# HansBambel/SmaAt-UNet

Hardware: NVIDIA H100
Metric: SmaAt-UNet fwd frames/sec @ B=32 12×288×288; depthwise % HBM roofline (higher is better)
Workload: dtype f32

## Files before the change

### smaat_unet_b200/csrc/dsconv_fused.cu

```cuda
#include <stdlib.h>

#include <type_traits>

#include "tc_common.cuh"

namespace smaat {

struct DsParams {
  const float* dw_w;
  const float* dw_b;
  const float* scale;
  const float* shift;
  float* y;
  int64_t y_bstride;
  double* stats;
  const float* oc_w;
  const float* oc_b;
  float* oc_y;
  const float* gate_sc;
  float* pool_sum;
  float* pool_max;
  float* pooled;
  int pooled_bf16;
  int npart;
// ... 301 lines not shown
        static_assert(GPC % 2 == 0, "fragment sets alternate within a chunk");
        const unsigned char* ast = nullptr;
        uint64_t bd = 0, bl = 0;
        AFrags<PREC, KS> fa, fb;
        auto step = [&](int i, int hf, int part, AFrags<PREC, KS>& cur, AFrags<PREC, KS>& prev) {
          if (part == 0) {
            if (hf == 0) {
              const int sa = gc % AS;
              mbar_wait(&a_full[sa], (gc / AS) & 1u);
              ast = a_base + sa * L::AST_BYTES;
            }
            wait_b(NW * gc + hf, bd, bl);
          }
          load_a_frags<PREC, KS>(ast, part * KS, t, m0, m1, cur);
          if (hf == 0) mma_a_frags<N_TILE, PREC, KS>(acc[0], cur, bd, bl, part * KS);
          else mma_a_frags<N_TILE, PREC, KS>(acc[NA - 1], cur, bd, bl, part * KS);
          wgmma_wait<1>();
          wgmma_keep(prev);
          if (part == 0) {
            if (hf == 1) release_b(NW * gc);
            else if (i > 0) release(gc - 1);
          }
        };
        for (int i = 0; i < nch; ++i, ++gc) {
#pragma unroll
          for (int hf = 0; hf < NW; ++hf) {
#pragma unroll
            for (int part = 0; part < GPC; part += 2) {
              step(i, hf, part, fa, fb);
              step(i, hf, part + 1, fb, fa);
            }
          }
        }
        wgmma_wait0();
        wgmma_keep(fa);
        wgmma_keep(fb);
      } else {
        constexpr int KS = L::KS, GPC = (TC_BK / 8) / KS;
        const unsigned char* ast = nullptr;
        uint64_t bd0 = 0, bl0 = 0;
        auto group = [&](AFrags<PREC, KS>(&cur)[NH], AFrags<PREC, KS>(&prev)[NH], int q) {
          const int part = q % GPC;
          if (part == 0) wait_stages(ast, bd0, bl0);
#pragma unroll
          for (int h = 0; h < NH; ++h) load_a_frags<PREC, KS>(ast + h * L::A_BYTES, part * KS, t, m0, m1, cur[h]);
          mma_a_frags<N_TILE, PREC, KS, NH>(acc, cur, bd0, bl0, part * KS);
          wgmma_wait<1>();
#pragma unroll
          for (int h = 0; h < NH; ++h) wgmma_keep(prev[h]);
          if (part == 0 && q > 0) release(gc - 1);
          if (part == GPC - 1) ++gc;
        };
        AFrags<PREC, KS> fa[NH], fb[NH];
        const int ngrp = nch * GPC;
        int q = 0;
        for (; q + 1 < ngrp; q += 2) {
          group(fa, fb, q);
          group(fb, fa, q + 1);
        }
        if (q < ngrp) group(fa, fb, q);
        wgmma_wait0();
#pragma unroll
        for (int h = 0; h < NH; ++h) {
          wgmma_keep(fa[h]);
          wgmma_keep(fb[h]);
        }
      }
#pragma unroll
      for (int h = 0; h < NA; ++h) wgmma_keep(acc[h]);
      release(gc - 1);

#pragma unroll
      for (int h = 0; h < NA; ++h) {
        float (&ac)[N_TILE / 2] = acc[h];
        const int hp = WIDE ? 0 : h;
        const int n0 = (np * NW + (WIDE ? h : 0)) * N_TILE;
        const int y_org = ty * TH + hp * PH;
        const int gy0 = y_org + m0 / PW, gx0 = tx * PW + m0 % PW;
        const int gy1 = y_org + m1 / PW, gx1 = tx * PW + m1 % PW;
        const bool v0 = gy0 < p.H && gx0 < p.W, v1 = gy1 < p.H && gx1 < p.W;
        const int64_t o0 = (int64_t)gy0 * p.W + gx0, o1 = (int64_t)gy1 * p.W + gx1;
        if (!WIDE && p.stats) {
          const double npix = (double)((__popc(__ballot_sync(0xffffffffu, v0)) + __popc(__ballot_sync(0xffffffffu, v1))) / 4);
#pragma unroll
          for (int j = 0; j < N_TILE / 8; ++j) {
#pragma unroll
            for (int e = 0; e < 2; ++e) {
              const float a = v0 ? ac[4 * j + e] : 0.f, bb = v1 ? ac[4 * j + 2 + e] : 0.f;
              const float s1 = frag_colsum(a + bb), s2 = frag_colsum(fmaf(a, a, bb * bb));
              const int c = 8 * j + 2 * t + e;
              if (lane < 4 && c < p.Cout) {
                const double sc = (double)aff[c], sh = (double)aff[L::AFF_N + c];
                atomicAdd(p.stats + c, sc * (double)s1 + npix * sh);
                atomicAdd(p.stats + p.Cout + c, sc * sc * (double)s2 + 2.0 * sc * sh * (double)s1 + npix * sh * sh);
              }
            }
          }
        }
        if (!WIDE && p.ncls) {
#pragma unroll
          for (int j = 0; j < N_TILE / 8; ++j) {
#pragma unroll
            for (int e = 0; e < 2; ++e) {
              const int c = 8 * j + 2 * t + e;
              const float sc = aff[c], sh = aff[L::AFF_N + c];
              ac[4 * j + e] = fmaxf(fmaf(ac[4 * j + e], sc, sh), act_lo);
              ac[4 * j + 2 + e] = fmaxf(fmaf(ac[4 * j + 2 + e], sc, sh), act_lo);
            }
          }
          float best0 = -INFINITY, best1 = -INFINITY;
          int arg0 = 0, arg1 = 0;
#pragma unroll 1
          for (int cl = 0; cl < p.ncls; ++cl) {
            const float* wr = cls_w + cl * N_TILE + 2 * t;
            float d0 = 0.f, d1 = 0.f;
#pragma unroll
            for (int j = 0; j < N_TILE / 8; ++j) {
              const float2 w = *reinterpret_cast<const float2*>(wr + 8 * j);
              d0 = fmaf(ac[4 * j], w.x, d0);
              d1 = fmaf(ac[4 * j + 2], w.x, d1);
              d0 = fmaf(ac[4 * j + 1], w.y, d0);
              d1 = fmaf(ac[4 * j + 3], w.y, d1);
            }
            d0 += __shfl_xor_sync(0xffffffffu, d0, 1);
            d0 += __shfl_xor_sync(0xffffffffu, d0, 2);
            d1 += __shfl_xor_sync(0xffffffffu, d1, 1);
            d1 += __shfl_xor_sync(0xffffffffu, d1, 2);
            const float ob = cls_b[cl];
            const float l0 = d0 + ob, l1 = d1 + ob;
            if (best0 == best0 && (l0 > best0 || l0 != l0)) { best0 = l0; arg0 = cl; }
            if (best1 == best1 && (l1 > best1 || l1 != l1)) { best1 = l1; arg1 = cl; }
            if (p.oc_y && t == (cl & 3)) {
              TA* yk = reinterpret_cast<TA*>(p.oc_y) + ((int64_t)b * p.ncls + cl) * P;
              if (v0) st_act(yk + o0, l0);
              if (v1) st_act(yk + o1, l1);
            }
          }
          if (p.cls) {
            if (v0 && t == 0) p.cls[(int64_t)b * P + o0] = arg0;
            if (v1 && t == 1) p.cls[(int64_t)b * P + o1] = arg1;
          }
        } else if (!WIDE && p.oc_y) {
          float d0 = 0.f, d1 = 0.f;
#pragma unroll
          for (int j = 0; j < N_TILE / 8; ++j) {
#pragma unroll
            for (int e = 0; e < 2; ++e) {
              const int c = 8 * j + 2 * t + e;
              const float sc = aff[c], sh = aff[L::AFF_N + c], w = aff[2 * L::AFF_N + c];
              d0 = fmaf(fmaxf(fmaf(ac[4 * j + e], sc, sh), act_lo), w, d0);
              d1 = fmaf(fmaxf(fmaf(ac[4 * j + 2 + e], sc, sh), act_lo), w, d1);
            }
          }
          d0 += __shfl_xor_sync(0xffffffffu, d0, 1);
          d0 += __shfl_xor_sync(0xffffffffu, d0, 2);
          d1 += __shfl_xor_sync(0xffffffffu, d1, 1);
          d1 += __shfl_xor_sync(0xffffffffu, d1, 2);
          const float ob = p.oc_b ? __ldg(p.oc_b) : 0.f;
          if (t == 0) {
            TA* oy = reinterpret_cast<TA*>(p.oc_y) + (int64_t)b * P;
            if (v0) st_act(oy + o0, d0 + ob);
            if (v1) st_act(oy + o1, d1 + ob);
          }
        } else if (L::ST_BUFS) {
          const int y_half = y_org + wg * (PH / 2);
#pragma unroll
          for (int s = 0; s < N_TILE / 32; ++s) {
            if (n0 + 32 * s >= p.Cout) break;
            const uint32_t buf = st_base + (st_n % L::ST_BUFS) * L::ST_BOX;
            if (st_leader) bulk_wait_read<L::ST_BUFS - 1>();
            wg_sync(2 + wg);
#pragma unroll
            for (int jj = 0; jj < 4; ++jj) {
              const int j = 4 * s + jj;
              float v[4];
#pragma unroll
              for (int q = 0; q < 4; ++q) v[q] = (t & 2) ? ac[4 * j + (q ^ 2)] : ac[4 * j + q];
              quad_transpose(v, quad);
              const int c = n0 + 8 * j + st_ch;
              const float sc = aff[c], sh = aff[L::AFF_N + c];
              const float4 o = make_float4(fmaxf(fmaf(v[0], sc, sh), act_lo), fmaxf(fmaf(v[1], sc, sh), act_lo),
                                           fmaxf(fmaf(v[2], sc, sh), act_lo), fmaxf(fmaf(v[3], sc, sh), act_lo));
              if constexpr (BA) {
                asm volatile("st.shared.v2.b32 [%0], {%1, %2};" ::"r"(buf + st_off + 1024u * jj), "r"(f32x2_bf16x2(o.x, o.y)),
                             "r"(f32x2_bf16x2(o.z, o.w))
                             : "memory");
              } else {
                asm volatile("st.shared.v4.f32 [%0], {%1, %2, %3, %4};" ::"r"(buf + st_off + 2048u * jj), "f"(o.x), "f"(o.y),
                             "f"(o.z), "f"(o.w)
                             : "memory");
              }
            }
            fence_proxy_async_smem();
            wg_sync(2 + wg);
            if (st_leader) {
              tma_store_4d(&map_y, buf, tx * PW, y_half, n0 + 32 * s, b);
              bulk_commit();
            }
            if (p.pooled) {
              const bool parts = !BA && p.pool_sum;
              const int pt = threadIdx.x & 127, pch = pt >> 2, pq = pt & 3;
              const int c = n0 + 32 * s + pch;
              float psum = 0.f, pmax = -INFINITY;
#pragma unroll
              for (int it = 0; it < 2; ++it) {
                constexpr int NQ = PW / 4;
                const int item = pq + 4 * it, rp = item / NQ, qd = item % NQ;
                const int px = 2 * rp * PW + 4 * qd;
                float4 u, v;
                if constexpr (BA) {
                  const uint32_t a0 = (uint32_t)(pch * 128 + px * 2), a1 = a0 + (uint32_t)(PW * 2);
                  uint2 hu, hv;
                  asm volatile("ld.shared.v2.b32 {%0, %1}, [%2];" : "=r"(hu.x), "=r"(hu.y) : "r"(buf + a0));
                  asm volatile("ld.shared.v2.b32 {%0, %1}, [%2];" : "=r"(hv.x), "=r"(hv.y) : "r"(buf + a1));
                  u = bf16x4_f32(hu);
                  v = bf16x4_f32(hv);
                } else {
                  const uint32_t a0 = (uint32_t)(pch * 256 + px * 4), a1 = a0 + (uint32_t)(PW * 4);
                  asm volatile("ld.shared.v4.f32 {%0, %1, %2, %3}, [%4];" : "=f"(u.x), "=f"(u.y), "=f"(u.z), "=f"(u.w)
                               : "r"(buf + (a0 ^ (((a0 >> 7) & SW_MASK) << 4))));
                  asm volatile("ld.shared.v4.f32 {%0, %1, %2, %3}, [%4];" : "=f"(v.x), "=f"(v.y), "=f"(v.z), "=f"(v.w)
                               : "r"(buf + (a1 ^ (((a1 >> 7) & SW_MASK) << 4))));
                }
                const int gy = y_half + 2 * rp, gx = tx * PW + 4 * qd;
                const bool in0 = gx < p.W && gy < p.H, in1 = gx < p.W && gy + 1 < p.H;
                if (parts && in0) {
                  psum += (u.x + u.y) + (u.z + u.w);
                  pmax = fmaxf(pmax, fmaxf(fmaxf(u.x, u.y), fmaxf(u.z, u.w)));
                }
                if (in1) {
                  if (parts) {
                    psum += (v.x + v.y) + (v.z + v.w);
                    pmax = fmaxf(pmax, fmaxf(fmaxf(v.x, v.y), fmaxf(v.z, v.w)));
                  }
                  if (c < p.Cout) {
                    const int hw = p.W >> 1;
                    const int64_t o = ((int64_t)b * p.Cout + c) * (int64_t)(p.H >> 1) * hw + (int64_t)(gy >> 1) * hw + (gx >> 1);
                    const float2 m2 = make_float2(fmaxf(fmaxf(u.x, u.y), fmaxf(v.x, v.y)), fmaxf(fmaxf(u.z, u.w), fmaxf(v.z, v.w)));
                    if (BA && p.pooled_bf16)
                      *reinterpret_cast<uint32_t*>(reinterpret_cast<uint16_t*>(p.pooled) + o) = f32x2_bf16x2(m2.x, m2.y);
                    else
                      *reinterpret_cast<float2*>(p.pooled + o) = m2;
                  }
                }
              }
              if (parts) {
                psum += __shfl_xor_sync(0xffffffffu, psum, 1);
                psum += __shfl_xor_sync(0xffffffffu, psum, 2);
                pmax = fmaxf(pmax, __shfl_xor_sync(0xffffffffu, pmax, 1));
                pmax = fmaxf(pmax, __shfl_xor_sync(0xffffffffu, pmax, 2));
                if (pq == 0 && c < p.Cout) {
                  const int64_t o = ((int64_t)b * p.npart + 2 * ((ty * NH + hp) * p.tiles_x + tx) + wg) * p.Cout + c;
                  p.pool_sum[o] = psum;
                  p.pool_max[o] = pmax;
                }
              }
            }
            ++st_n;
          }
        } else {
          TA* yb = reinterpret_cast<TA*>(p.y) + (int64_t)b * p.y_bstride;
#pragma unroll
          for (int j = 0; j < N_TILE / 8; ++j) {
#pragma unroll
            for (int e = 0; e < 2; ++e) {
              const int c = n0 + 8 * j + 2 * t + e;
              if (c < p.Cout) {
                const float sc = aff[c], sh = aff[L::AFF_N + c];
                TA* yc = yb + (int64_t)c * P;
                if (v0) st_act(yc + o0, fmaxf(fmaf(ac[4 * j + e], sc, sh), act_lo));
                if (v1) st_act(yc + o1, fmaxf(fmaf(ac[4 * j + 2 + e], sc, sh), act_lo));
              }
            }
          }
        }
      }
    }
    if (L::ST_BUFS && st_leader) bulk_wait_all();
    return;
  }

  {
    if (L::REGS_PROD < L::REGS_LAUNCH) regs_dealloc<L::REGS_PROD>();
    const int g = (warp - L::PROD_WARP) >> 2;
    const int t = threadIdx.x - 32 * L::PROD_WARP - 128 * g;
    const int Cin = p.C0 + p.C1;
    constexpr int KH = KPL == 4 ? 2 : KPL, NT = CC * 8;
    const int kr0 = KH == KPL ? 0 : t / NT * KH;
    const float* dw_w = p.dw_w + kr0 * 9;
    const float* dw_b = p.dw_b ? p.dw_b + kr0 : nullptr;
    uint32_t gc = 0, iph = 0;
    for (int tile = blockIdx.x; tile < p.total_tiles; tile += gridDim.x) {
      const int b = tile / tiles_per_img;
      for (int i = 0; i < nch; ++i, ++gc) {
        if ((int)(gc % (uint32_t)L::NG) != g) continue;
        const int s = gc % IS;
        const bool gated = p.gate_sc && i * CC < p.C0;
        auto task_base = [&](int task) { return KH == KPL ? task : task & (NT - 1); };
        float wr[KH][9], br[KH], gsc = 0.f;
        auto task_channel = [&](int task) { return (PW == 32) ? (task >> 3) : (((task >> 4) << 1) | ((task >> 2) & 1)); };
        auto load_weights = [&](int task) {
          const int gch = i * CC + task_channel(task_base(task));
          const bool chv = gch < Cin;
#pragma unroll
          for (int kk = 0; kk < KH; ++kk) {
            const int gk = gch * KPL + kk;
#pragma unroll
            for (int w9 = 0; w9 < 9; ++w9) wr[kk][w9] = chv ? __ldg(dw_w + (int64_t)gk * 9 + w9) : 0.f;
            br[kk] = (chv && dw_b) ? __ldg(dw_b + gk) : 0.f;
          }
          if (gated) gsc = gch < p.C0 ? __ldg(p.gate_sc + (int64_t)b * p.C0 + gch) : 0.f;
        };
        load_weights(t);
        mbar_wait(&in_full[s * L::NG + g], (iph >> s) & 1u);
        iph ^= 1u << s;
        const int sa = gc % AS;
        mbar_wait(&a_empty[sa], ((gc / AS) & 1u) ^ 1u);
        unsigned char* my_op = a_base + sa * L::AST_BYTES;
        const TA* in_stage = reinterpret_cast<const TA*>(smem + s * L::IN_BYTES);
        const float* sa_stage = reinterpret_cast<const float*>(smem + L::OFF_SA + s * L::SA_BYTES);
        auto stencil = [&](auto gate_c) {
          constexpr bool G = decltype(gate_c)::value;
#pragma unroll 1
          for (int task = t; task < NT * (KPL / KH); task += 128) {
            const int tb = task_base(task);
            int ci, qc, rg;
            if (PW == 32) {
              ci = tb >> 3; qc = tb & 7; rg = 0;
            } else {
              qc = tb & 3; ci = ((tb >> 4) << 1) | ((tb >> 2) & 1); rg = (tb >> 3) & 1;
            }
            constexpr int NQ = PW / 4;
            const int c0 = qc << 2, r0 = rg << 2;
            if (task != t) load_weights(task);
            const TA* trow = in_stage + (ci * BH + r0) * BW + c0 + L::XM - 1;
            const float* srow = sa_stage + r0 * BW + c0 + L::XM - 1;
            float win[3][6];
            const bool lb = (qc == 0), rb = (qc == NQ - 1);
            const int edge = lb ? 0 : 5;
            auto load_row = [&](float* wl, int r) {
              float4 a;
              if constexpr (BA) a = bf16x4_f32(*reinterpret_cast<const uint2*>(trow + r * BW + 1));
              else a = *reinterpret_cast<const float4*>(trow + r * BW + 1);
              if (G) {
                const float4 ga = *reinterpret_cast<const float4*>(srow + r * BW + 1);
                a.x = __fmul_rn(__fmul_rn(a.x, gsc), ga.x);
                a.y = __fmul_rn(__fmul_rn(a.y, gsc), ga.y);
                a.z = __fmul_rn(__fmul_rn(a.z, gsc), ga.z);
                a.w = __fmul_rn(__fmul_rn(a.w, gsc), ga.w);
              }
              float left = __shfl_up_sync(0xffffffffu, a.w, 1), right = __shfl_down_sync(0xffffffffu, a.x, 1);
              if (lb | rb) {
                float e;
                if constexpr (BA) e = bf16_f32(trow[r * BW + edge]);
                else e = trow[r * BW + edge];
                if (G) e = __fmul_rn(__fmul_rn(e, gsc), srow[r * BW + edge]);
                if (lb) left = e; else right = e;
              }
              wl[0] = left; wl[1] = a.x; wl[2] = a.y; wl[3] = a.z; wl[4] = a.w; wl[5] = right;
            };
#pragma unroll
            for (int h = 0; h < NH; ++h) {
#pragma unroll
              for (int r = 0; r < 2; ++r) load_row(win[r], h * PH + r);
#pragma unroll
              for (int rr = 0; rr < 4; ++rr) {
                load_row(win[(rr + 2) % 3], h * PH + rr + 2);
                const float* w0 = win[rr % 3];
                const float* w1 = win[(rr + 1) % 3];
                const float* w2 = win[(rr + 2) % 3];
                const int m = (r0 + rr) * PW + c0;
#pragma unroll
                for (int kk = 0; kk < KH; ++kk) {
                  float o4[4];
#pragma unroll
                  for (int j = 0; j < 4; ++j) {
                    float a = br[kk];
                    a = fmaf(wr[kk][0], w0[j], a); a = fmaf(wr[kk][1], w0[j + 1], a); a = fmaf(wr[kk][2], w0[j + 2], a);
                    a = fmaf(wr[kk][3], w1[j], a); a = fmaf(wr[kk][4], w1[j + 1], a); a = fmaf(wr[kk][5], w1[j + 2], a);
                    a = fmaf(wr[kk][6], w2[j], a); a = fmaf(wr[kk][7], w2[j + 1], a); a = fmaf(wr[kk][8], w2[j + 2], a);
                    o4[j] = a;
                  }
                  if (A_SMEM) {
                    const int kr = ci * KPL + kr0 + kk;
#pragma unroll
                    for (int j = 0; j < 4; ++j) {
                      const uint32_t off = kmajor_offset(m + j, kr);
                      const float hi = X3 ? tf32_hi(o4[j]) : o4[j];
                      *reinterpret_cast<float*>(my_op + off) = hi;
                      if (X3) *reinterpret_cast<float*>(my_op + L::OFF_ALO + off) = o4[j] - hi;
                    }
                    continue;
                  }
                  *reinterpret_cast<float4*>(my_op + h * L::A_BYTES + a_tile_offset(ci * KPL + kr0 + kk, m)) =
                      make_float4(o4[0], o4[1], o4[2], o4[3]);
                }
              }
            }
          }
        };
        if (gated) stencil(std::true_type{}); else stencil(std::false_type{});
        if (A_SMEM) fence_proxy_async_smem();
        mbar_arrive(&a_full[sa]);
        mbar_arrive(&in_empty[s]);
      }
    }
  }
}

__host__ __device__ constexpr Prec tf32_prec(bool x3) { return x3 ? Prec::TF32X3 : Prec::TF32; }

template <int N_TILE, int KPL, int PW, bool X3, bool A_SMEM>
__global__ void __launch_bounds__(DsCfg<N_TILE, KPL, PW, tf32_prec(X3), A_SMEM>::THREADS, 1)
    dsconv_fused_kernel(const __grid_constant__ CUtensorMap map_in0, const __grid_constant__ CUtensorMap map_in1,
                        const __grid_constant__ CUtensorMap map_w, const __grid_constant__ CUtensorMap map_wlo,
                        const __grid_constant__ CUtensorMap map_y, const __grid_constant__ CUtensorMap map_sa,
                        const DsParams p) {
  dsconv_body<N_TILE, KPL, PW, tf32_prec(X3), A_SMEM>(map_in0, map_in1, map_w, map_wlo, map_y, map_sa, p);
}

template <int N_TILE, int PW, bool X3>
__global__ void __launch_bounds__(DsCfg<N_TILE, 4, PW, tf32_prec(X3), false>::THREADS, 1)
    dsconv_kpl4_kernel(const __grid_constant__ CUtensorMap map_in0, const __grid_constant__ CUtensorMap map_in1,
                       const __grid_constant__ CUtensorMap map_w, const __grid_constant__ CUtensorMap map_wlo,
                       const __grid_constant__ CUtensorMap map_y, const __grid_constant__ CUtensorMap map_sa,
                       const DsParams p) {
  dsconv_body<N_TILE, 4, PW, tf32_prec(X3), false>(map_in0, map_in1, map_w, map_wlo, map_y, map_sa, p);
}

template <int N_TILE, int KPL, int PW>
__global__ void __launch_bounds__(DsCfg<N_TILE, KPL, PW, Prec::BF16, false>::THREADS, 1)
    dsconv_bf16_kernel(const __grid_constant__ CUtensorMap map_in0, const __grid_constant__ CUtensorMap map_in1,
                       const __grid_constant__ CUtensorMap map_w, const __grid_constant__ CUtensorMap map_wlo,
                       const __grid_constant__ CUtensorMap map_y, const __grid_constant__ CUtensorMap map_sa,
                       const DsParams p) {
  dsconv_body<N_TILE, KPL, PW, Prec::BF16, false>(map_in0, map_in1, map_w, map_wlo, map_y, map_sa, p);
}

template <int N_TILE, int KPL, int PW>
__global__ void __launch_bounds__(DsCfg<N_TILE, KPL, PW, Prec::BF16, false, uint16_t>::THREADS, 1)
    dsconv_bf16act_kernel(const __grid_constant__ CUtensorMap map_in0, const __grid_constant__ CUtensorMap map_in1,
                          const __grid_constant__ CUtensorMap map_w, const __grid_constant__ CUtensorMap map_wlo,
                          const __grid_constant__ CUtensorMap map_y, const __grid_constant__ CUtensorMap map_sa,
                          const DsParams p) {
  dsconv_body<N_TILE, KPL, PW, Prec::BF16, false, uint16_t>(map_in0, map_in1, map_w, map_wlo, map_y, map_sa, p);
}

template <int KPL, int PW, bool X3>
__global__ void __launch_bounds__(DsCfg<64, KPL, PW, tf32_prec(X3), false, float, true>::THREADS, 1)
    dsconv_pair_kernel(const __grid_constant__ CUtensorMap map_in0, const __grid_constant__ CUtensorMap map_in1,
                       const __grid_constant__ CUtensorMap map_w, const __grid_constant__ CUtensorMap map_wlo,
                       const __grid_constant__ CUtensorMap map_y, const __grid_constant__ CUtensorMap map_sa,
                       const DsParams p) {
  dsconv_body<64, KPL, PW, tf32_prec(X3), false, float, true>(map_in0, map_in1, map_w, map_wlo, map_y, map_sa, p);
}

template <int PW, bool X3>
__global__ void __launch_bounds__(DsCfg<128, 2, PW, tf32_prec(X3), false, float, false, true>::THREADS, 1)
    dsconv_wide_kernel(const __grid_constant__ CUtensorMap map_in0, const __grid_constant__ CUtensorMap map_in1,
                       const __grid_constant__ CUtensorMap map_w, const __grid_constant__ CUtensorMap map_wlo,
                       const __grid_constant__ CUtensorMap map_y, const __grid_constant__ CUtensorMap map_sa,
                       const DsParams p) {
  dsconv_body<128, 2, PW, tf32_prec(X3), false, float, false, true>(map_in0, map_in1, map_w, map_wlo, map_y, map_sa, p);
}

template <int N_TILE, int KPL, int PW, Prec P, bool A_SMEM, typename TA = float, bool PAIR = false, bool WIDE = false>
static auto ds_kernel() {
  static_assert(KPL == 1 || KPL == 2 || (KPL == 4 && !A_SMEM), "fused DS conv instances: k = 1, 2 (both A forms), 4 (register form)");
  if constexpr (WIDE) return dsconv_wide_kernel<PW, P == Prec::TF32X3>;
  else if constexpr (PAIR) return dsconv_pair_kernel<KPL, PW, P == Prec::TF32X3>;
  else if constexpr (sizeof(TA) == 2) return dsconv_bf16act_kernel<N_TILE, KPL, PW>;
  else if constexpr (P == Prec::BF16) return dsconv_bf16_kernel<N_TILE, KPL, PW>;
  else if constexpr (KPL == 4) return dsconv_kpl4_kernel<N_TILE, PW, P == Prec::TF32X3>;
  else return dsconv_fused_kernel<N_TILE, KPL, PW, P == Prec::TF32X3, A_SMEM>;
}

template <int N_TILE, int KPL, int PW, Prec P, bool A_SMEM, typename TA, bool PAIR, bool WIDE>
static int launch_ds(DsCfg<N_TILE, KPL, PW, P, A_SMEM, TA, PAIR, WIDE>, const CUtensorMap& m0, const CUtensorMap& m1,
                     const CUtensorMap& mw, const CUtensorMap& mwl, const CUtensorMap& my, const CUtensorMap& msa, DsParams p, int B,
                     cudaStream_t st) {
  using L = DsCfg<N_TILE, KPL, PW, P, A_SMEM, TA, PAIR, WIDE>;
  auto kern = ds_kernel<N_TILE, KPL, PW, P, A_SMEM, TA, PAIR, WIDE>();
  static std::atomic<uint64_t> attr_mask{0};
  if (first_use_on_device(attr_mask)) {
    cudaError_t e = cudaFuncSetAttribute(kern, cudaFuncAttributeMaxDynamicSharedMemorySize, L::TOTAL + L::CLS_SMEM);
    if (e != cudaSuccess)
      return fail(SMAAT_E_CUDA, "dsconv: smem attribute (%d B): %s", L::TOTAL + L::CLS_SMEM, cudaGetErrorString(e));
    int r = check_reg_budget((const void*)kern, L::THREADS, L::REGS_SUM, "dsconv");
    if (r) return r;
  }
  p.tiles_x = ceil_div(p.W, PW);
  p.tiles_y = ceil_div(p.H, L::TH);
  p.npass = ceil_div(p.Cout, N_TILE * L::NW);
  const int64_t total = (int64_t)B * p.tiles_x * p.tiles_y * p.npass;
  SMAAT_REQUIRE(total < (1ll << 31), "dsconv: too many tiles");
  p.total_tiles = (int)total;
  p.nchunks = ceil_div(p.C0 + p.C1, L::CC);
  p.npart = 2 * p.tiles_x * p.tiles_y * L::NH;
  const int grid = p.total_tiles < num_sms() ? p.total_tiles : num_sms();
  kern<<<grid, L::THREADS, L::TOTAL + (p.ncls ? L::CLS_SMEM : 0), st>>>(m0, m1, mw, mwl, my, msa, p);
  SMAAT_LAUNCH_CHECK("smaat_dsconv_fwd");
  return SMAAT_OK;
}

static int pick_pw(int H, int W) {
  double best = 1e9;
  int pw = 0;
  const int cand[2] = {32, 16};
  for (int i = 0; i < 2; ++i) {
    const int c = cand[i], ph = TC_BM / c;
    const double waste = ((double)ceil_div(W, c) * c / W) * ((double)ceil_div(H, ph) * ph / H);
    if (waste < best - 1e-9) {
      best = waste;
      pw = c;
    }
  }
  return best <= 1.35 ? pw : 0;
}

static std::atomic<int> g_ds_impl{-1};
static int ds_impl() {
  int v = g_ds_impl.load(std::memory_order_relaxed);
  if (v < 0) {
    const char* e = getenv("SMAAT_DS_IMPL");
    v = e ? atoi(e) : 0;
    if (v < 0 || v > 2) v = 0;
    g_ds_impl.store(v, std::memory_order_relaxed);
  }
  return v;
}

static std::atomic<int> g_ds_wide{-1};
static bool ds_wide_on() {
  int v = g_ds_wide.load(std::memory_order_relaxed);
  if (v < 0) {
    const char* e = getenv("SMAAT_DSCONV_WIDE");
    v = (e && atoi(e) == 0) ? 0 : 1;
    g_ds_wide.store(v, std::memory_order_relaxed);
  }
  return v != 0;
}

static std::atomic<int> g_ds_pair{-1};
static bool ds_pair_on() {
  int v = g_ds_pair.load(std::memory_order_relaxed);
  if (v < 0) {
    const char* e = getenv("SMAAT_DSCONV_PAIR");
    v = (e && atoi(e) == 0) ? 0 : 1;
    g_ds_pair.store(v, std::memory_order_relaxed);
  }
  return v != 0;
}

struct DsReq {
  const void* x0; int C0; int64_t x0_bstride;
  const void* x1; int C1; int64_t x1_bstride;
  const void* pw_w; int H, W, k, Cout;
  int B = 0, relu = 0, mode = SMAAT_PW_TF32;
  bool bact = false;
  const float* dw_w = nullptr; const float* dw_b = nullptr; const float* pw_w_lo = nullptr;
  const float* scale = nullptr; const float* shift = nullptr;
  void* y = nullptr; int64_t y_bstride = 0;
  double* stats = nullptr;
  const float* oc_w = nullptr; const float* oc_b = nullptr;
  void* oc_y = nullptr; int ncls = 0; int64_t* cls = nullptr;
  const float* gate_sc = nullptr; const float* gate_sa = nullptr;
  float* pool_sum = nullptr; float* pool_max = nullptr;
  void* pooled = nullptr; int pooled_bf16 = 0;
  bool head() const { return oc_y || ncls > 0; }
};

alignas(16) static char g_ds_asked[16];

enum DsDecline { DS_TAKEN, DS_SHAPE, DS_UNSTAGED, DS_CLASSES };
struct DsInst {
  int n_tile, k, pw;
  Prec prec;
  bool a_smem, bact, pair, wide;
  DsDecline declined;
};

template <int N_TILE, int KPL, int PW, Prec P, typename F>
static int ds_visit_inst(const DsInst& c, F& f) {
  if constexpr (P != Prec::BF16 && N_TILE == 128 && KPL == 2) {
    if (c.wide) return f(DsCfg<128, 2, PW, P, false, float, false, true>{});
  }
  if constexpr (P != Prec::BF16 && N_TILE == 64 && KPL != 1) {
    if (c.pair) return f(DsCfg<64, KPL, PW, P, false, float, true>{});
  }
  if constexpr (P == Prec::BF16 && KPL != 4) {
    if (c.bact) return f(DsCfg<N_TILE, KPL, PW, P, false, uint16_t>{});
  }
  if constexpr (P != Prec::BF16 && KPL != 4) {
    if (c.a_smem) return f(DsCfg<N_TILE, KPL, PW, P, true>{});
  }
  return f(DsCfg<N_TILE, KPL, PW, P, false>{});
}
template <int N_TILE, int KPL, int PW, typename F>
static int ds_visit_prec(const DsInst& c, F& f) {
  if (c.prec == Prec::BF16) return ds_visit_inst<N_TILE, KPL, PW, Prec::BF16>(c, f);
  if (c.prec == Prec::TF32X3) return ds_visit_inst<N_TILE, KPL, PW, Prec::TF32X3>(c, f);
  return ds_visit_inst<N_TILE, KPL, PW, Prec::TF32>(c, f);
}
template <typename F>
static int ds_visit(const DsInst& c, F f) {
  if (c.n_tile == 64) {
    if (c.k == 4) return c.pw == 32 ? ds_visit_prec<64, 4, 32>(c, f) : ds_visit_prec<64, 4, 16>(c, f);
    if (c.k == 2) return c.pw == 32 ? ds_visit_prec<64, 2, 32>(c, f) : ds_visit_prec<64, 2, 16>(c, f);
    return c.pw == 32 ? ds_visit_prec<64, 1, 32>(c, f) : ds_visit_prec<64, 1, 16>(c, f);
  }
  if (c.k == 4) return c.pw == 32 ? ds_visit_prec<128, 4, 32>(c, f) : ds_visit_prec<128, 4, 16>(c, f);
  if (c.k == 2) return c.pw == 32 ? ds_visit_prec<128, 2, 32>(c, f) : ds_visit_prec<128, 2, 16>(c, f);
  return c.pw == 32 ? ds_visit_prec<128, 1, 32>(c, f) : ds_visit_prec<128, 1, 16>(c, f);
}

static int ds_max_classes(const DsInst& c) {
  return ds_visit(c, [](auto cfg) { return (int)decltype(cfg)::MAX_CLASSES; });
}

static DsInst ds_select(const DsReq& r) {
  const bool a_smem = ds_impl() == 1, bf16 = r.mode == SMAAT_PW_BF16, head = r.head(), stats = r.stats;
  const int k = r.k, Cout = r.Cout;
  const Prec prec = bf16 ? Prec::BF16 : r.mode == SMAAT_PW_TF32X3 ? Prec::TF32X3 : Prec::TF32;
  DsInst c{Cout > 64 ? 128 : 64, k, pick_pw(r.H, r.W), prec, a_smem, r.bact, false, false, DS_SHAPE};
  if ((k != 1 && k != 2 && k != 4) || (a_smem && (k == 4 || bf16))) return c;
  if (r.bact && (!bf16 || k == 4 || stats || r.W % 8 != 0 || r.x0_bstride % 8 != 0 || (r.C1 > 0 && r.x1_bstride % 8 != 0) ||
                 (r.y && r.y_bstride % 8 != 0)))
    return c;
  if (r.y && (!aligned16(r.y) || r.y_bstride % 4 != 0)) return c;
  c.wide = ds_wide_on() && Cout > 128 && Cout <= 256 && k == 2 && !a_smem && !bf16 && !head;
  if (Cout < 8 || Cout > 512 || (Cout > 128 && (stats || head))) return c;
  if (Cout > 128 && Cout % 128 != 0 && !c.wide) return c;
  if (r.W % 4 != 0 || !aligned16(r.x0) || r.x0_bstride % 4 != 0) return c;
  if (r.C1 > 0 && (!aligned16(r.x1) || r.x1_bstride % 4 != 0 || r.C0 % (TC_BK / k) != 0)) return c;
  if ((k * (r.C0 + r.C1) % 4 != 0 && !r.bact) || !aligned16(r.pw_w) || (r.pw_w_lo && !aligned16(r.pw_w_lo))) return c;
  if (!c.pw) return c;
  c.pair = ds_pair_on() && c.n_tile == 64 && (k == 2 || k == 4) && !a_smem && !bf16 && ceil_div(r.H, TC_BM / c.pw) % 2 == 0 &&
           r.ncls <= DS_MIN_CLASSES;
  const bool staged = ds_visit(c, [](auto cfg) { return (int)decltype(cfg)::ST_BUFS; }) > 0;
  c.declined = r.pooled && !staged ? DS_UNSTAGED : r.ncls > ds_max_classes(c) ? DS_CLASSES : DS_TAKEN;
  return c;
}

static int ds_launch(const DsReq& r, void* stream) {
  const int B = r.B, C0 = r.C0, C1 = r.C1, H = r.H, W = r.W, k = r.k, Cout = r.Cout;
  const bool head = r.head(), bf16 = r.mode == SMAAT_PW_BF16;
  SMAAT_REQUIRE(r.x0 && r.dw_w && r.pw_w && (r.y || r.oc_y || r.cls), "dsconv: null pointer");
  SMAAT_REQUIRE(!r.gate_sc == !r.gate_sa, "dsconv: the CBAM gate needs both sc and sa");
  SMAAT_REQUIRE(!r.gate_sa || aligned16(r.gate_sa), "dsconv: the CBAM gate map must be 16-byte aligned");
  SMAAT_REQUIRE(!r.pool_sum || (r.pool_max && r.pooled && r.y && !r.oc_y && !r.stats),
                "dsconv: the CBAM pools need sum, max and max-pool outputs and y");
  SMAAT_REQUIRE(!r.pooled || (r.y && !head && !r.stats), "dsconv: the max-pool needs y, and no OutConv or batch statistics");
  SMAAT_REQUIRE(!r.pooled_bf16 || r.bact, "dsconv: a bf16 max-pool needs bf16 activations");
  SMAAT_REQUIRE(!r.pooled || (reinterpret_cast<uintptr_t>(r.pooled) & (r.pooled_bf16 ? 3u : 7u)) == 0,
                "dsconv: the max-pool output must be %d-byte aligned", r.pooled_bf16 ? 4 : 8);
  SMAAT_REQUIRE(B > 0 && C0 > 0 && C1 >= 0 && H > 0 && W > 0 && Cout > 0, "dsconv: bad shape");
  SMAAT_REQUIRE(C1 == 0 || r.x1, "dsconv: C1=%d but x1 is null", C1);
  SMAAT_REQUIRE(r.mode == SMAAT_PW_TF32 || r.mode == SMAAT_PW_TF32X3 || r.mode == SMAAT_PW_BF16,
                "dsconv: mode must be SMAAT_PW_TF32, SMAAT_PW_TF32X3 or SMAAT_PW_BF16");
  SMAAT_REQUIRE(r.mode != SMAAT_PW_TF32X3 || r.pw_w_lo, "dsconv: TF32X3 needs pw_w_lo (see smaat_split_tf32)");
  SMAAT_REQUIRE(head || r.y_bstride >= (int64_t)Cout * H * W, "dsconv: y batch stride too small");
  SMAAT_REQUIRE(!head || (r.oc_w && !r.stats), "dsconv+outconv: needs the OutConv weight and no batch statistics");
  SMAAT_REQUIRE(!r.bact || (bf16 && !r.stats && !r.pool_sum), "dsconv: bf16 activations take bf16 operands, no statistics and no pools");
  const DsInst c = ds_select(r);
  if (c.declined == DS_SHAPE)
    return fail(SMAAT_E_UNSUPPORTED,
                r.bact ? "dsconv_bf16: not taken by the bf16-activation kernel (k=%d Cout=%d H=%d W=%d; needs k = 1 or 2, W and the "
                         "batch strides multiples of 8, 16-byte aligned tensors, the register A form)"
                       : "dsconv: shape or output layout not taken by the fused kernel (k=%d Cout=%d H=%d W=%d, y 16-byte aligned "
                         "with a batch stride that is a multiple of 4); use dw3x3 + pw1x1",
                k, Cout, H, W);
  if (c.declined == DS_UNSTAGED)
    return fail(SMAAT_E_UNSUPPORTED, "dsconv: the CBAM pools and the max-pool need the staged epilogue");
  if (c.declined == DS_CLASSES)
    return fail(SMAAT_E_UNSUPPORTED, "dsconv+classify: %d classes, this instance keeps the weights of at most %d", r.ncls,
                ds_max_classes(c));
  const int pw = c.pw, ph = TC_BM / pw, cc = TC_BK / k, K = k * (C0 + C1);
  const int th = c.pair ? 2 * ph : ph;
  const CUtensorMapDataType adt = r.bact ? CU_TENSOR_MAP_DATA_TYPE_BFLOAT16 : CU_TENSOR_MAP_DATA_TYPE_FLOAT32;
  const uint64_t esz = r.bact ? 2 : 4;

  CUtensorMap m0, m1, mw, mwl;
  const int xm = 16 / (int)esz;
  const uint32_t box[4] = {(uint32_t)(pw + 2 * xm), (uint32_t)(th + 2), (uint32_t)cc, 1u};
  {
    const uint64_t dims[4] = {(uint64_t)W, (uint64_t)H, (uint64_t)C0, (uint64_t)B};
    const uint64_t str[4] = {0, (uint64_t)W * esz, (uint64_t)H * W * esz, (uint64_t)r.x0_bstride * esz};
    int e = make_tmap(&m0, adt, r.x0, 4, dims, str, box, CU_TENSOR_MAP_SWIZZLE_NONE, "dsconv(x0)");
    if (e) return e;
    m1 = m0;
  }
  if (C1 > 0) {
    const uint64_t dims[4] = {(uint64_t)W, (uint64_t)H, (uint64_t)C1, (uint64_t)B};
    const uint64_t str[4] = {0, (uint64_t)W * esz, (uint64_t)H * W * esz, (uint64_t)r.x1_bstride * esz};
    int e = make_tmap(&m1, adt, r.x1, 4, dims, str, box, CU_TENSOR_MAP_SWIZZLE_NONE, "dsconv(x1)");
    if (e) return e;
  }
  {
    const uint64_t kw = bf16 ? (uint64_t)(K + TC_BK - 1) / TC_BK * TC_BK : (uint64_t)K;
// ... 232 lines not shown
```

Baseline: 2894.

## Stream depthwise stencil rows continuously across sub-tiles with precomputed store offsets

The depthwise 3x3 stencil now runs one continuous sliding window over all NH*4 rows of a task. It no longer restarts at each PH sub-tile and reloads two halo rows each time. The A-operand store offsets are precomputed once per kernel row and adjusted with XOR/add arithmetic instead of calling a_tile_offset per store. Weight addressing goes through a single base pointer pinned with an empty asm statement. The task-to-row mapping also changes (r0 = rg*NR), which alters work assignment and raises register pressure from the 4-row window.

```diff
diff --git a/smaat_unet_b200/csrc/dsconv_fused.cu b/smaat_unet_b200/csrc/dsconv_fused.cu
--- a/smaat_unet_b200/csrc/dsconv_fused.cu
+++ b/smaat_unet_b200/csrc/dsconv_fused.cu
@@ -627,12 +627,13 @@
         auto load_weights = [&](int task) {
           const int gch = i * CC + task_channel(task_base(task));
           const bool chv = gch < Cin;
+          const float* wk = dw_w + gch * (KPL * 9);
+          asm("" : "+l"(wk));
 #pragma unroll
           for (int kk = 0; kk < KH; ++kk) {
-            const int gk = gch * KPL + kk;
-#pragma unroll
-            for (int w9 = 0; w9 < 9; ++w9) wr[kk][w9] = chv ? __ldg(dw_w + (int64_t)gk * 9 + w9) : 0.f;
-            br[kk] = (chv && dw_b) ? __ldg(dw_b + gk) : 0.f;
+#pragma unroll
+            for (int w9 = 0; w9 < 9; ++w9) wr[kk][w9] = chv ? __ldg(wk + kk * 9 + w9) : 0.f;
+            br[kk] = (chv && dw_b) ? __ldg(dw_b + gch * KPL + kk) : 0.f;
           }
           if (gated) gsc = gch < p.C0 ? __ldg(p.gate_sc + (int64_t)b * p.C0 + gch) : 0.f;
         };
@@ -656,13 +657,12 @@
               qc = tb & 3; ci = ((tb >> 4) << 1) | ((tb >> 2) & 1); rg = (tb >> 3) & 1;
             }
             constexpr int NQ = PW / 4;
-            const int c0 = qc << 2, r0 = rg << 2;
+            constexpr int NR = 4 * NH;
+            const int c0 = qc << 2, r0 = rg * NR;
             if (task != t) load_weights(task);
             const TA* trow = in_stage + (ci * BH + r0) * BW + c0 + L::XM - 1;
             const float* srow = sa_stage + r0 * BW + c0 + L::XM - 1;
-            float win[3][6];
             const bool lb = (qc == 0), rb = (qc == NQ - 1);
-            const int edge = lb ? 0 : 5;
             auto load_row = [&](float* wl, int r) {
               float4 a;
               if constexpr (BA) a = bf16x4_f32(*reinterpret_cast<const uint2*>(trow + r * BW + 1));
@@ -675,51 +675,56 @@
                 a.w = __fmul_rn(__fmul_rn(a.w, gsc), ga.w);
               }
               float left = __shfl_up_sync(0xffffffffu, a.w, 1), right = __shfl_down_sync(0xffffffffu, a.x, 1);
-              if (lb | rb) {
+              auto halo = [&](int c) {
                 float e;
-                if constexpr (BA) e = bf16_f32(trow[r * BW + edge]);
-                else e = trow[r * BW + edge];
-                if (G) e = __fmul_rn(__fmul_rn(e, gsc), srow[r * BW + edge]);
-                if (lb) left = e; else right = e;
-              }
+                if constexpr (BA) e = bf16_f32(trow[r * BW + c]);
+                else e = trow[r * BW + c];
+                if (G) e = __fmul_rn(__fmul_rn(e, gsc), srow[r * BW + c]);
+                return e;
+              };
+              if (lb) left = halo(0);
+              if (rb) right = halo(5);
               wl[0] = left; wl[1] = a.x; wl[2] = a.y; wl[3] = a.z; wl[4] = a.w; wl[5] = right;
             };
-#pragma unroll
-            for (int h = 0; h < NH; ++h) {
-#pragma unroll
-              for (int r = 0; r < 2; ++r) load_row(win[r], h * PH + r);
-#pragma unroll
-              for (int rr = 0; rr < 4; ++rr) {
-                load_row(win[(rr + 2) % 3], h * PH + rr + 2);
-                const float* w0 = win[rr % 3];
-                const float* w1 = win[(rr + 1) % 3];
-                const float* w2 = win[(rr + 2) % 3];
-                const int m = (r0 + rr) * PW + c0;
-#pragma unroll
-                for (int kk = 0; kk < KH; ++kk) {
-                  float o4[4];
+            uint32_t ao[KH];
+#pragma unroll
+            for (int kk = 0; kk < KH; ++kk)
+              ao[kk] = (uint32_t)((r0 / PH) * L::A_BYTES) + a_tile_offset(ci * KPL + kr0 + kk, (r0 % PH) * PW + c0);
+            float win[4][6];
+#pragma unroll
+            for (int r = 0; r < 3; ++r) load_row(win[r], r);
+#pragma unroll
+            for (int rr = 0; rr < NR; ++rr) {
+              if (rr + 3 < NR + 2) load_row(win[(rr + 3) % 4], rr + 3);
+              const float* w0 = win[rr % 4];
+              const float* w1 = win[(rr + 1) % 4];
+              const float* w2 = win[(rr + 2) % 4];
+              const int m = (r0 % PH + rr % PH) * PW + c0;
+#pragma unroll
+              for (int kk = 0; kk < KH; ++kk) {
+                float o4[4];
+#pragma unroll
+                for (int j = 0; j < 4; ++j) {
+                  float a = br[kk];
+                  a = fmaf(wr[kk][0], w0[j], a); a = fmaf(wr[kk][1], w0[j + 1], a); a = fmaf(wr[kk][2], w0[j + 2], a);
+                  a = fmaf(wr[kk][3], w1[j], a); a = fmaf(wr[kk][4], w1[j + 1], a); a = fmaf(wr[kk][5], w1[j + 2], a);
+                  a = fmaf(wr[kk][6], w2[j], a); a = fmaf(wr[kk][7], w2[j + 1], a); a = fmaf(wr[kk][8], w2[j + 2], a);
+                  o4[j] = a;
+                }
+                if (A_SMEM) {
+                  const int kr = ci * KPL + kr0 + kk;
 #pragma unroll
                   for (int j = 0; j < 4; ++j) {
-                    float a = br[kk];
-                    a = fmaf(wr[kk][0], w0[j], a); a = fmaf(wr[kk][1], w0[j + 1], a); a = fmaf(wr[kk][2], w0[j + 2], a);
-                    a = fmaf(wr[kk][3], w1[j], a); a = fmaf(wr[kk][4], w1[j + 1], a); a = fmaf(wr[kk][5], w1[j + 2], a);
-                    a = fmaf(wr[kk][6], w2[j], a); a = fmaf(wr[kk][7], w2[j + 1], a); a = fmaf(wr[kk][8], w2[j + 2], a);
-                    o4[j] = a;
+                    const uint32_t off = kmajor_offset(m + j, kr);
+                    const float hi = X3 ? tf32_hi(o4[j]) : o4[j];
+                    *reinterpret_cast<float*>(my_op + off) = hi;
+                    if (X3) *reinterpret_cast<float*>(my_op + L::OFF_ALO + off) = o4[j] - hi;
                   }
-                  if (A_SMEM) {
-                    const int kr = ci * KPL + kr0 + kk;
-#pragma unroll
-                    for (int j = 0; j < 4; ++j) {
-                      const uint32_t off = kmajor_offset(m + j, kr);
-                      const float hi = X3 ? tf32_hi(o4[j]) : o4[j];
-                      *reinterpret_cast<float*>(my_op + off) = hi;
-                      if (X3) *reinterpret_cast<float*>(my_op + L::OFF_ALO + off) = o4[j] - hi;
-                    }
-                    continue;
-                  }
-                  *reinterpret_cast<float4*>(my_op + h * L::A_BYTES + a_tile_offset(ci * KPL + kr0 + kk, m)) =
-                      make_float4(o4[0], o4[1], o4[2], o4[3]);
+                  continue;
                 }
+                const int d = (rr % PH) * PW;
+                const uint32_t off = ((d & 16) ? ao[kk] ^ 64u : ao[kk]) + (uint32_t)((rr / PH) * L::A_BYTES + (d >> 5) * (TC_BK * 128));
+                *reinterpret_cast<float4*>(my_op + off) = make_float4(o4[0], o4[1], o4[2], o4[3]);
               }
             }
           }
```

After: 2970 (median of 6 runs). +2.6%, better.
